# EdwardLiuyc/StaticMapping

Hardware: AMD Instinct MI355X
Metric: scan-pair alignments/sec (120k-pt KITTI-64, 20 ICP iters) (higher is better)
Workload: dtype f32/f64; 1 GPU; BASELINE config #2: IcpFast point-to-plane, 120k-pt synthetic Velodyne-64 scan pair vs CalculateNormals target (~21695 pts), exactly 20 iterations, rho 0.7; 512 distinct consecutive pairs of a synthetic drive (speed 6-10 m/s, yaw rate +-0.2 rad/s, seed 5), guess = previous pair's motion; pairs_per_gpu=512, distinct_pairs=512, target_points_mean=21695, nn_mode=grid, guess=extrapolated, split_after=2, parallelism=pairs round-robin over 1 GPU(s), one RCCL gather of poses, rccl_ranks=1

## Files before the change

### staticmapping_amd/csrc/icp_kernels.hip

```cpp
#include <type_traits>
#include "smhip_device.h"
#include "kd_median_tree.h"
#include "grid_lookup.h"
#include "icp_tail_math.h"

namespace smhip {

__device__ __forceinline__ bool xcd_block(int nblk, int npairs, int b_pair_base, int& pair, int& blk) {
  const int id = blockIdx.x;
  const int j = id >> 3;
  const int local = (j / nblk) * 8 + (id & 7);
  pair = b_pair_base + local;
  blk = j % nblk;
  return local < npairs;
}

__global__ __launch_bounds__(256) void tgt_reduce(IcpDev b) {
  const int pair = b.pair_base + blockIdx.y;
  const int nt = b.in[pair].nt;
  const float4* tp = b.tgt_p + (size_t)pair * b.nt_cap;
  double sx = 0, sy = 0, sz = 0;
  float mn[3] = {INFINITY, INFINITY, INFINITY}, mx[3] = {-INFINITY, -INFINITY, -INFINITY};
  const int chunk = (nt + gridDim.x - 1) / gridDim.x;
  const int lo = blockIdx.x * chunk, hi = min(nt, lo + chunk);
// ... 640 lines not shown
    unsigned long long m[4];
    if (!class_masks(it, m)) continue;
#pragma unroll
    for (int c = 0; c < 4; ++c) tot[c] += (uint32_t)__popcll(m[c]);
  }
  uint32_t basepos[4];
#pragma unroll
  for (int c = 0; c < 4; ++c) {
    uint32_t v = 0;
    if (lane == 0 && tot[c]) v = atomicAdd(&st->nabo_count[c], tot[c]);
    basepos[c] = (uint32_t)__builtin_amdgcn_readlane((int)v, 0);
  }
#pragma unroll
  for (int it = 0; it < ITEMS; ++it) {
    unsigned long long m[4];
    if (!class_masks(it, m)) continue;
    const uint32_t c = (uint32_t)(cls2 >> (2 * it)) & 3u;
    if ((nabo_failed >> it) & 1u) {
      const unsigned long long mine = c == 0 ? m[0] : (c == 1 ? m[1] : (c == 2 ? m[2] : m[3]));
      const uint32_t bp = c == 0 ? basepos[0] : (c == 1 ? basepos[1] : (c == 2 ? basepos[2] : basepos[3]));
      *nabo_list_slot(b, so, (int)c, bp + (uint32_t)__popcll(mine & lt)) = base + it * kNnThreads + (int)threadIdx.x;
    }
#pragma unroll
    for (int c2 = 0; c2 < 4; ++c2) basepos[c2] += (uint32_t)__popcll(m[c2]);
  }
}

template <int ITEMS, bool NABO = false>
__global__ __launch_bounds__(kNnThreads) void nn_certify(IcpDev b, int nblk) {
  int pair, blk;
  if (!xcd_block(nblk, b.npairs, b.pair_base, pair, blk)) return;
  PairState* st = &b.state[pair];
  if (st->done) return;
  const int ns = st->ns;
  const int base = blk * (kNnThreads * ITEMS);
  if (base >= ns) return;
  double Mc[12];
#pragma unroll
  for (int k = 0; k < 12; ++k) Mc[k] = st->M[k];
  const Pot pot = {(float)st->pot_a, (float)st->pot_b, 0.f, 0.f};
  __shared__ uint32_t s_hist[kHistBins];
  for (int k = threadIdx.x; k < kHistBins; k += kNnThreads) s_hist[k] = 0;
  __syncthreads();
  const int lane = threadIdx.x & 63;
  const size_t so = (size_t)pair * b.ns_cap;
  const float4* __restrict__ tq = b.tq + (size_t)pair * b.nt_cap;
  const float r_need = 0.9f * sqrtf(st->rcap2);
  uint32_t min_lb = 0xffffffffu;
  uint32_t nabo_failed = 0;
  int ic = min(base + (int)threadIdx.x, ns - 1);
  float4 s_1 = ld_src(b, so + ic);
  float l_1 = ld_lb(b, so + ic);
  int j_1 = b.idx[so + ic];
  ic = min(base + kNnThreads + (int)threadIdx.x, ns - 1);
  float4 s_2 = ld_src(b, so + ic);
  float l_2 = ld_lb(b, so + ic);
  int j_2 = b.idx[so + ic];
  float4 t_1 = tq[max(j_1, 0)];
  for (int it = 0; it < ITEMS; ++it) {
    const int i = base + it * kNnThreads + threadIdx.x;
    bool hard = false, fail = false;
    const float4 s = s_1;
    const float l = l_1;
    const int j = j_1;
    const float4 t = t_1;
    s_1 = s_2; l_1 = l_2; j_1 = j_2;
    if (it + 1 < ITEMS) t_1 = tq[max(j_1, 0)];
    if (it + 2 < ITEMS) {
      ic = min(i + 2 * kNnThreads, ns - 1);
      s_2 = ld_src(b, so + ic);
      l_2 = ld_lb(b, so + ic);
      j_2 = b.idx[so + ic];
    }
    if (i < ns) {
      double px, py, pz;
      transform_point(Mc, s, px, py, pz);
      const float qx = (float)px, qy = (float)py, qz = (float)pz;
      const float Lp = bound_now(l, pot_at(pot, norm3(s.x, s.y, s.z)));
      fail = true;
      if (NABO) {
        const float Pn = pot_at(pot, norm3(s.x, s.y, s.z));
        if (isfinite(qx) && isfinite(qy) && isfinite(qz) && l > 0.f && j >= 0 &&
            l - Pn - 4.0e-7f * (l + Pn) - 1.3e-7f * (fabsf(qx) + fabsf(qy) + fabsf(qz)) > 0.f) {
          const float d1 = dist2(t, qx, qy, qz);
          b.d2[so + i] = d1;
          atomicAdd(&s_hist[__float_as_uint(d1) >> kHistShift], 1u);
          fail = false;
        }
      } else if (isfinite(qx) && isfinite(qy) && isfinite(qz) && Lp > 0.f) {
        if (l > 0.f && j >= 0) {
          const float d1 = dist2(t, qx, qy, qz);
          if (d1 < Lp * Lp) {
            b.d2[so + i] = d1;
            atomicAdd(&s_hist[__float_as_uint(d1) >> kHistShift], 1u);
            fail = false;
          }
        } else if (l < 0.f && Lp >= r_need) {
          const float lb2 = Lp * Lp;
          b.d2[so + i] = lb2;
          atomicAdd(&s_hist[__float_as_uint(lb2) >> kHistShift], 1u);
          min_lb = min(min_lb, __float_as_uint(lb2));
          hard = true;
          fail = false;
        }
      }
    }
    const unsigned long long dm = __ballot(fail);
    if (NABO) {
      if (fail) nabo_failed |= 1u << it;
    } else if (dm) {
      uint32_t basepos = 0;
      if (lane == 0) basepos = atomicAdd(&st->deferred_count, (uint32_t)__popcll(dm));
      basepos = (uint32_t)__builtin_amdgcn_readlane((int)basepos, 0);
      if (fail) b.dlist[so + basepos + __popcll(dm & ((1ull << lane) - 1ull))] = i;
    }
    const unsigned long long hm = __ballot(hard);
    if (hm) {
      uint32_t basepos = 0;
      if (lane == 0) basepos = atomicAdd(&st->hard_count, (uint32_t)__popcll(hm));
      basepos = (uint32_t)__builtin_amdgcn_readlane((int)basepos, 0);
      if (hard) b.hlist[so + basepos + __popcll(hm & ((1ull << lane) - 1ull))] = i;
    }
  }
  if (NABO) nabo_list_append<ITEMS>(b, st, so, base, ns, nabo_failed, lane);
#pragma unroll
  for (int off = 32; off > 0; off >>= 1) min_lb = min(min_lb, (uint32_t)__shfl_xor((int)min_lb, off, 64));
  if (lane == 0 && min_lb != 0xffffffffu) atomicMin(&st->min_lb_key, min_lb);
  __syncthreads();
  uint32_t* gh = b.hist + (size_t)pair * kHistBins;
  for (int k = threadIdx.x; k < kHistBins; k += kNnThreads) {
    const uint32_t v = s_hist[k];
    if (v) atomicAdd(&gh[k], v);
  }
}

__device__ __forceinline__ void sweep_run(const float4* __restrict__ tq, uint32_t j0, uint32_t j1,
                                          float qx, float qy, float qz, Best& best) {
  uint32_t j = j0;
  for (; j + 4 <= j1; j += 4) {
    const float4 t0 = tq[j], t1 = tq[j + 1], t2 = tq[j + 2], t3 = tq[j + 3];
    test_ascending_ru(t0, (int)j, qx, qy, qz, best);
    test_ascending_ru(t1, (int)j + 1, qx, qy, qz, best);
    test_ascending_ru(t2, (int)j + 2, qx, qy, qz, best);
    test_ascending_ru(t3, (int)j + 3, qx, qy, qz, best);
  }
  for (; j < j1; ++j) test_ascending_ru(tq[j], (int)j, qx, qy, qz, best);
}

#ifndef SMHIP_PHASE_TIMING
#define SMHIP_PHASE_TIMING 0
#endif
#if SMHIP_PHASE_TIMING
#define SMHIP_PHASE(k) do { if (timing) { const unsigned long long now_ = __builtin_readcyclecounter(); tacc[k] += now_ - tprev; tprev = now_; } } while (0)
#else
#define SMHIP_PHASE(k) do { } while (0)
#endif
template <int ITEMS, bool FIRST>
__device__ __forceinline__ void ball_lds_rounds(const IcpDev& b, PairState* st, const PairState* ls, int pair, int base0, const double* Mc,
                                                uint32_t* s_hist, uint32_t& min_lb) {
  const int ns = ls->ns;
  const Pot pot = {(float)ls->pot_a, (float)ls->pot_b, (float)ls->step_a, (float)ls->step_b};
  const float Mtx = (float)Mc[3], Mty = (float)Mc[7], Mtz = (float)Mc[11];
#if SMHIP_PHASE_TIMING
  const bool timing = (b.debug_flags & 16) != 0;
  unsigned long long tacc[8] = {0, 0, 0, 0, 0, 0, 0, 0};
  unsigned long long tprev = timing ? __builtin_readcyclecounter() : 0ull;
#endif
  __shared__ uint32_t s_tab[kLdsTableCap];
  __shared__ float4 s_pts[kLdsPointCap];
  __shared__ uint32_t s_roff[kLdsRowCap + 1];
  __shared__ uint32_t s_occ[kLdsRowCap / 32 + 1];
  __shared__ float4 s_q[kNnThreads];
  __shared__ float s_r2[kNnThreads];
  __shared__ uint16_t s_lid[kNnThreads];
  __shared__ uint32_t s_nsearch[2];
  __shared__ uint32_t s_w[17];
  __shared__ int s_box[2][6];
  if (threadIdx.x < 6) { s_box[0][threadIdx.x] = threadIdx.x < 3 ? 0x3fffffff : -0x3fffffff; s_box[1][threadIdx.x] = s_box[0][threadIdx.x]; }
  if (threadIdx.x < 2) s_nsearch[threadIdx.x] = 0;
  __syncthreads();
  const int lane = threadIdx.x & 63;
  const size_t so = (size_t)pair * b.ns_cap;
  const uint2* __restrict__ words = b.words + (size_t)pair * kMaxGridWords;
  const uint32_t* __restrict__ cstart = b.cstart + (size_t)pair * (b.nt_cap + 1);
  const float4* __restrict__ tq = b.tq + (size_t)pair * b.nt_cap;
  const float ox = ls->origin[0], oy = ls->origin[1], oz = ls->origin[2];
  const float h = ls->h, inv_h = ls->inv_h;
  const int nx = ls->nx, ny = ls->ny, nz = ls->nz, wx = ls->wx, nw = ls->nw;
  const float r2cap = ls->rcap2;
  const float r_need = 0.9f * sqrtf(r2cap);
  const bool have_prev = !FIRST && ls->iter > 0;
  const bool certify = have_prev && b.certify;

  int i = base0 + threadIdx.x;
  float4 s_cur = make_float4(0, 0, 0, 0);
  int jp_cur = -1;
  float l_cur = 0.f;
  if (i < ns) {
    s_cur = ld_src(b, so + i);
    if (have_prev) { jp_cur = b.idx[so + i]; if (certify) l_cur = ld_lb(b, so + i); }
  }

  for (int it = 0; it < ITEMS; ++it) {
    const int base = base0 + it * kNnThreads;
    if (base >= ns) break;
    i = base + threadIdx.x;
    int* box = s_box[it & 1];
    uint32_t* nsearch = &s_nsearch[it & 1];
    const int i_next = i + kNnThreads;
    float4 s_next = make_float4(0, 0, 0, 0);
    int jp_next = -1;
    float l_next = 0.f;
    if (it + 1 < ITEMS && i_next < ns) {
      s_next = ld_src(b, so + i_next);
      if (have_prev) { jp_next = b.idx[so + i_next]; if (certify) l_next = ld_lb(b, so + i_next); }
    }
    SMHIP_PHASE(0);
    float qx = 0.f, qy = 0.f, qz = 0.f;
    bool valid = false;
    if (i < ns) {
      double px, py, pz;
      transform_point(Mc, s_cur, px, py, pz);
      qx = (float)px; qy = (float)py; qz = (float)pz;
      valid = isfinite(qx) && isfinite(qy) && isfinite(qz);
    }
    const bool has_jp = valid && jp_cur >= 0;
    float dub2 = INFINITY;
    if (has_jp) dub2 = dist2(tq[jp_cur], qx, qy, qz);
    bool need_search = valid, hard = false;
    if (i < ns && !valid) {
      b.d2[so + i] = INFINITY; st_match(b, so + i, -1, 0.f);
    }
    const float sn = __builtin_amdgcn_sqrtf(fmaf(s_cur.z, s_cur.z, fmaf(s_cur.y, s_cur.y, s_cur.x * s_cur.x)));
    const float delta = have_prev ? fmaf(pot.sa, sn, pot.sb) : 0.03f;
    if (certify && valid) {
      const float Lp = bound_now(l_cur, pot_at(pot, sn));
      if (Lp > 0.f) {
        if (l_cur > 0.f && has_jp && dub2 < Lp * Lp) {
          b.d2[so + i] = dub2;
          atomicAdd(&s_hist[__float_as_uint(dub2) >> kHistShift], 1u);
          need_search = false;
        } else if (l_cur < 0.f && Lp >= r_need) {
          const float lb2 = Lp * Lp;
          b.d2[so + i] = lb2;
          atomicAdd(&s_hist[__float_as_uint(lb2) >> kHistShift], 1u);
          min_lb = min(min_lb, __float_as_uint(lb2));
          hard = true;
          need_search = false;
        }
      }
    }
    {
      const unsigned long long sm = __ballot(need_search);
      if (sm) {
        uint32_t basepos = 0;
        if (lane == 0) basepos = atomicAdd(nsearch, (uint32_t)__popcll(sm));
        basepos = (uint32_t)__builtin_amdgcn_readlane((int)basepos, 0);
        if (need_search) {
          const uint32_t pos = basepos + __popcll(sm & ((1ull << lane) - 1ull));
          s_q[pos] = make_float4(qx, qy, qz, __int_as_float(jp_cur));
          s_r2[pos] = has_jp ? search_radius2(r2cap, dub2, search_margin(delta)) : r2cap;
          s_lid[pos] = (uint16_t)threadIdx.x;
        }
      }
    }
    {
      const unsigned long long hm = __ballot(hard);
      if (hm) {
        uint32_t basepos = 0;
        if (lane == 0) basepos = atomicAdd(&st->hard_count, (uint32_t)__popcll(hm));
        basepos = (uint32_t)__builtin_amdgcn_readlane((int)basepos, 0);
        if (hard) b.hlist[so + basepos + __popcll(hm & ((1ull << lane) - 1ull))] = i;
      }
    }
    SMHIP_PHASE(1);
    __syncthreads();
    SMHIP_PHASE(2);
    const int nq = (int)*nsearch;
    if (threadIdx.x == 0 && nq) atomicAdd(&st->deferred_count, (uint32_t)nq);
    const bool mine = (int)threadIdx.x < nq;
    float R2 = 0.f;
    int jseed = -1, gi = -1;
    if (mine) {
      const float4 q4 = s_q[threadIdx.x];
      qx = q4.x; qy = q4.y; qz = q4.z; jseed = __float_as_int(q4.w);
      R2 = s_r2[threadIdx.x];
      gi = base + (int)s_lid[threadIdx.x];
    }
    int x0 = 1, x1 = 0, y0 = 1, y1 = 0, z0 = 1, z1 = 0;
    if (mine) {
      const float Rs = __builtin_amdgcn_sqrtf(R2) * 1.0001f + 1.0e-3f * h;
      x0 = max(cell_coord(qx - Rs, ox, inv_h), 0); x1 = min(cell_coord(qx + Rs, ox, inv_h), nx - 1);
      y0 = max(cell_coord(qy - Rs, oy, inv_h), 0); y1 = min(cell_coord(qy + Rs, oy, inv_h), ny - 1);
      z0 = max(cell_coord(qz - Rs, oz, inv_h), 0); z1 = min(cell_coord(qz + Rs, oz, inv_h), nz - 1);
    }
    const bool inbox = mine && x0 <= x1 && y0 <= y1 && z0 <= z1;
    if ((int)(threadIdx.x & ~63) < nq) {
      const int big = 0x3fffffff;
      const int mx0 = wave_min_i(inbox ? x0 : big), mx1 = wave_max_i(inbox ? x1 : -big);
      const int my0 = wave_min_i(inbox ? y0 : big), my1 = wave_max_i(inbox ? y1 : -big);
      const int mz0 = wave_min_i(inbox ? z0 : big), mz1 = wave_max_i(inbox ? z1 : -big);
      if (lane == 0 && mx0 <= mx1) {
        atomicMin(&box[0], mx0); atomicMin(&box[1], my0); atomicMin(&box[2], mz0);
        atomicMax(&box[3], mx1); atomicMax(&box[4], my1); atomicMax(&box[5], mz1);
      }
    }
    SMHIP_PHASE(3);
    __syncthreads();
    const int X0 = box[0], Y0 = box[1], Z0 = box[2];
    const int nxl = box[3] - X0 + 2, nyl = box[4] - Y0 + 1, nzl = box[5] - Z0 + 1;
    const bool any = box[3] >= X0;
    const long long entries = any ? (long long)nxl * nyl * nzl : 0;
    const bool use_lds = any && entries <= kLdsTableCap;
    if (use_lds) {
      const float inv_nxl = 1.0f / (float)nxl, inv_nyl = 1.0f / (float)nyl;
      for (int e = threadIdx.x; e < (int)entries; e += kNnThreads) {
        const int r = (int)(((float)e + 0.5f) * inv_nxl);
        const int x = X0 + (e - r * nxl);
        const int zz = (int)(((float)r + 0.5f) * inv_nyl);
        const int y = Y0 + (r - zz * nyl), z = Z0 + zz;
        const int widx = (z * ny + y) * wx + (x >> 5);
        uint32_t val = (uint32_t)ls->nt;
        if (widx < nw) {
          const uint2 wd = words[widx];
          val = cstart[wd.y + __popc(wd.x & ((1u << (x & 31)) - 1u))];
        }
        s_tab[e] = val;
      }
    }
    if (threadIdx.x < 6) s_box[(it + 1) & 1][threadIdx.x] = threadIdx.x < 3 ? 0x3fffffff : -0x3fffffff;
    if (threadIdx.x == 6) s_nsearch[(it + 1) & 1] = 0;
    const int rows = use_lds ? nyl * nzl : 0;
    bool pts_lds = use_lds && rows <= kLdsRowCap;
    if (use_lds) __syncthreads();
    if (pts_lds) {
      uint32_t len = 0;
      if ((int)threadIdx.x < rows) len = s_tab[threadIdx.x * nxl + nxl - 1] - s_tab[threadIdx.x * nxl];
      {
        const unsigned long long om = __ballot(len > 0);
        if (lane == 0) { s_occ[2 * (threadIdx.x >> 6)] = (uint32_t)om; s_occ[2 * (threadIdx.x >> 6) + 1] = (uint32_t)(om >> 32); }
        if (threadIdx.x == 0) s_occ[kLdsRowCap / 32] = 0u;
      }
      uint32_t total;
      const uint32_t off = block_excl_scan(len, s_w, &total);
      if ((int)threadIdx.x < rows) s_roff[threadIdx.x] = off;
      if (threadIdx.x == 0) s_roff[rows] = total;
      __syncthreads();
      pts_lds = total <= (uint32_t)kLdsPointCap;
      if (pts_lds) {
        for (uint32_t k = threadIdx.x; k < total; k += kNnThreads) {
          int lo = 0, hi = rows - 1;
          while (lo < hi) { const int mid = (lo + hi + 1) >> 1; if (s_roff[mid] <= k) lo = mid; else hi = mid - 1; }
          const uint32_t j = s_tab[lo * nxl] + (k - s_roff[lo]);
          float4 t = tq[j];
          t.w = __int_as_float((int)j);
          s_pts[k] = t;
        }
      }
    }
    __syncthreads();
    SMHIP_PHASE(4);
    bool hard2 = false;
    if (mine) {
      Best best = {INFINITY, -1, INFINITY};
      if (x0 <= x1 && y0 <= y1 && z0 <= z1) {
        const float slack = 2.0e-3f * h;
        const uint32_t ymask = (2u << (y1 - y0)) - 1u;
        for (int z = z0; z <= z1; ++z) {
          const float zl = oz + (float)z * h;
          const float dz = fmaxf(fmaxf(zl - qz, qz - (zl + h)) - slack, 0.f);
          const int ra = (z - Z0) * nyl + (y0 - Y0);
          uint32_t m = ymask;
          if (pts_lds) m &= __builtin_amdgcn_alignbit(s_occ[(ra >> 5) + 1], s_occ[ra >> 5], (uint32_t)(ra & 31));
          while (m) {
            const int bpos = __ffs((int)m) - 1;
            m &= m - 1u;
            const int y = y0 + bpos;
            const float yl = oy + (float)y * h;
            const float dy = fmaxf(fmaxf(yl - qy, qy - (yl + h)) - slack, 0.f);
            if (fmaf(dy, dy, dz * dz) > R2) continue;
            if (pts_lds) {
              const int r = ra + bpos;
              const int rb = r * nxl - X0;
              const uint32_t g0 = s_tab[rb + X0];
              const uint32_t k0 = s_roff[r] + (s_tab[rb + x0] - g0), k1 = s_roff[r] + (s_tab[rb + x1 + 1] - g0);
              for (const float4 *tp = s_pts + k0, *te = s_pts + k1; tp < te; ++tp) {
                const float4 t = *tp;
                test_ascending_ru(t, __float_as_int(t.w), qx, qy, qz, best);
              }
            } else if (use_lds) {
              const int rb = (ra + bpos) * nxl - X0;
              sweep_run(tq, s_tab[rb + x0], s_tab[rb + x1 + 1], qx, qy, qz, best);
            } else {
              uint32_t sb, se;
              row_slots(words, (z * ny + y) * wx, x0, x1, sb, se);
              if (se > sb) sweep_run(tq, cstart[sb], cstart[se], qx, qy, qz, best);
            }
          }
        }
      }
      float d2out, lbout;
      int jout;
      if (best.d2 <= R2) {
        d2out = best.d2;
        jout = best.j;
        lbout = __builtin_amdgcn_sqrtf(fminf(best.s2, R2));
      } else {
        d2out = R2;
        jout = best.j >= 0 ? best.j : jseed;
        lbout = -__builtin_amdgcn_sqrtf(R2);
        hard2 = true;
        min_lb = min(min_lb, __float_as_uint(R2));
      }
      SMHIP_PHASE(5);
      b.d2[so + gi] = d2out;
      {
        const float ux = qx - Mtx, uy = qy - Mty, uz = qz - Mtz;
        st_match(b, so + gi, jout, with_pot(lbout, pot_at(pot, __builtin_amdgcn_sqrtf(fmaf(uz, uz, fmaf(uy, uy, ux * ux))))));
      }
      const uint32_t key = __float_as_uint(d2out);
      if (key < 0x7f800000u) atomicAdd(&s_hist[key >> kHistShift], 1u);
    }
    {
      const unsigned long long hm = __ballot(hard2);
      if (hm) {
        uint32_t basepos = 0;
        if (lane == 0) basepos = atomicAdd(&st->hard_count, (uint32_t)__popcll(hm));
        basepos = (uint32_t)__builtin_amdgcn_readlane((int)basepos, 0);
        if (hard2) b.hlist[so + basepos + __popcll(hm & ((1ull << lane) - 1ull))] = gi;
      }
    }
    s_cur = s_next; jp_cur = jp_next; l_cur = l_next;
    SMHIP_PHASE(6);
  }
#if SMHIP_PHASE_TIMING
  if (timing && lane == 0) {
    unsigned long long* tc = reinterpret_cast<unsigned long long*>(b.tpart);
    for (int k = 0; k < 8; ++k) atomicAdd(&tc[k], tacc[k]);
  }
#endif
}

__device__ __forceinline__ void flush_min_lb(PairState* st, uint32_t min_lb) {
#pragma unroll
  for (int off = 32; off > 0; off >>= 1) min_lb = min(min_lb, (uint32_t)__shfl_xor((int)min_lb, off, 64));
  if ((threadIdx.x & 63) == 0 && min_lb != 0xffffffffu) atomicMin(&st->min_lb_key, min_lb);
}
__device__ __forceinline__ void flush_hist(const IcpDev& b, int pair, const uint32_t* s_hist) {
  __syncthreads();
  uint32_t* gh = b.hist + (size_t)pair * kHistBins;
  for (int k = threadIdx.x; k < kHistBins; k += kNnThreads) {
    const uint32_t v = s_hist[k];
    if (v) atomicAdd(&gh[k], v);
  }
}
__device__ __forceinline__ void flush_min_lb_and_hist(const IcpDev& b, PairState* st, int pair, uint32_t min_lb, const uint32_t* s_hist) {
  flush_min_lb(st, min_lb);
  flush_hist(b, pair, s_hist);
}

template <int ITEMS, bool FIRST = false>
__global__ __launch_bounds__(kNnThreads, 5) void nn_ball_lds(IcpDev b, int nblk) {
  int pair, blk;
  if (!xcd_block(nblk, b.npairs, b.pair_base, pair, blk)) return;
  PairState* st = &b.state[pair];
  if (st->done) return;
  const int base0 = blk * (kNnThreads * ITEMS);
  if (base0 >= st->ns) return;
  double Mc[12];
#pragma unroll
  for (int k = 0; k < 12; ++k) Mc[k] = st->M[k];
  __shared__ uint32_t s_hist[kHistBins];
  for (int k = threadIdx.x; k < kHistBins; k += kNnThreads) s_hist[k] = 0;
  uint32_t min_lb = 0xffffffffu;
  ball_lds_rounds<ITEMS, FIRST>(b, st, st, pair, base0, Mc, s_hist, min_lb);
  flush_min_lb_and_hist(b, st, pair, min_lb, s_hist);
}

__device__ __forceinline__ void listed_append_hard(const IcpDev& b, PairState* st, size_t so, bool hard, int i, int lane);
constexpr int kWaveBoxRows = 1024;
constexpr int kWaveCand = 256;

__device__ __forceinline__ void lane_ball_search(const uint2* __restrict__ words, const uint32_t* __restrict__ cstart, const float4* __restrict__ tq,
                                                 float ox, float oy, float oz, float h, int ny, int wx, float qx, float qy, float qz, float R2,
                                                 int x0, int x1, int y0, int y1, int z0, int z1, Best& best) {
  const float slack = 2.0e-3f * h;
  for (int z = z0; z <= z1; ++z) {
    const float zl = oz + (float)z * h;
    const float dz = fmaxf(fmaxf(zl - qz, qz - (zl + h)) - slack, 0.f);
    for (int y = y0; y <= y1; ++y) {
      const float yl = oy + (float)y * h;
      const float dy = fmaxf(fmaxf(yl - qy, qy - (yl + h)) - slack, 0.f);
      if (fmaf(dy, dy, dz * dz) > R2) continue;
      uint32_t sb, se;
      row_slots(words, (z * ny + y) * wx, x0, x1, sb, se);
      if (se > sb) {
        const uint32_t j0 = cstart[sb], j1 = cstart[se];
        for (uint32_t j = j0; j < j1; ++j) test_ascending_ru(tq[j], (int)j, qx, qy, qz, best);
      }
    }
  }
}
__device__ __forceinline__ void test_pair_ru(const float4 a, const float4 c, float qx, float qy, float qz, Best& best) {
  const f32x2 dx = (f32x2){qx, qx} - (f32x2){a.x, a.y};
  const f32x2 dy = (f32x2){qy, qy} - (f32x2){a.z, a.w};
  const f32x2 dz = (f32x2){qz, qz} - (f32x2){c.x, c.y};
  f32x2 d = dx * dx;
  d = __builtin_elementwise_fma(dy, dy, d);
  d = __builtin_elementwise_fma(dz, dz, d);
  best.s2 = __builtin_amdgcn_fmed3f(d.x, best.d2, best.s2);
  if (d.x < best.d2) { best.d2 = d.x; best.j = __float_as_int(c.z); }
  best.s2 = __builtin_amdgcn_fmed3f(d.y, best.d2, best.s2);
  if (d.y < best.d2) { best.d2 = d.y; best.j = __float_as_int(c.w); }
}

template <int ITEMS, bool FIRST>
__global__ __launch_bounds__(kNnThreads) void nn_ball_wave(IcpDev b, int nblk) {
  int pair, blk;
  if (!xcd_block(nblk, b.npairs, b.pair_base, pair, blk)) return;
  PairState* st = &b.state[pair];
  if (st->done) return;
  const int ns = st->ns;
  const int base0 = blk * (kNnThreads * ITEMS);
  if (base0 >= ns) return;
  double Mc[12];
#pragma unroll
  for (int k = 0; k < 12; ++k) Mc[k] = st->M[k];
  const Pot pot = {(float)st->pot_a, (float)st->pot_b, (float)st->step_a, (float)st->step_b};
  const float Mtx = (float)Mc[3], Mty = (float)Mc[7], Mtz = (float)Mc[11];
  __shared__ uint32_t s_hist[kHistBins];
  __shared__ float4 s_cand[kNnThreads / 64][kWaveCand];
  __shared__ uint32_t s_roff[kNnThreads / 64][64];
  __shared__ uint32_t s_rbase[kNnThreads / 64][64];
  __shared__ uint32_t s_nsearch;
  for (int k = threadIdx.x; k < kHistBins; k += kNnThreads) s_hist[k] = 0;
  if (threadIdx.x == 0) s_nsearch = 0;
  __syncthreads();
  const int lane = threadIdx.x & 63, wave = threadIdx.x >> 6;
  float4* cand = s_cand[wave];
  uint32_t* roff = s_roff[wave];
  uint32_t* rbase = s_rbase[wave];
  const size_t so = (size_t)pair * b.ns_cap;
  const uint2* __restrict__ words = b.words + (size_t)pair * kMaxGridWords;
  const uint32_t* __restrict__ cstart = b.cstart + (size_t)pair * (b.nt_cap + 1);
  const float4* __restrict__ tq = b.tq + (size_t)pair * b.nt_cap;
  const float ox = st->origin[0], oy = st->origin[1], oz = st->origin[2];
  const float h = st->h, inv_h = st->inv_h;
  const int nx = st->nx, ny = st->ny, nz = st->nz, wx = st->wx;
  const float r2cap = st->rcap2;
  const float r_need = 0.9f * sqrtf(r2cap);
  const bool have_prev = !FIRST && st->iter > 0;
  const bool certify = have_prev && b.certify;
  uint32_t min_lb = 0xffffffffu;
  uint32_t nsearch = 0;

  int i = base0 + threadIdx.x;
  float4 s_cur = make_float4(0, 0, 0, 0);
  int jp_cur = -1;
  float l_cur = 0.f;
  if (i < ns) {
    s_cur = ld_src(b, so + i);
    if (have_prev) { jp_cur = b.idx[so + i]; if (certify) l_cur = ld_lb(b, so + i); }
  }
  for (int it = 0; it < ITEMS; ++it) {
    const int base = base0 + it * kNnThreads;
    if (base >= ns) break;
    i = base + threadIdx.x;
    const int i_next = i + kNnThreads;
    float4 s_next = make_float4(0, 0, 0, 0);
    int jp_next = -1;
    float l_next = 0.f;
    if (it + 1 < ITEMS && i_next < ns) {
      s_next = ld_src(b, so + i_next);
      if (have_prev) { jp_next = b.idx[so + i_next]; if (certify) l_next = ld_lb(b, so + i_next); }
    }
    float qx = 0.f, qy = 0.f, qz = 0.f;
    bool valid = false;
    if (i < ns) {
      double px, py, pz;
      transform_point(Mc, s_cur, px, py, pz);
      qx = (float)px; qy = (float)py; qz = (float)pz;
      valid = isfinite(qx) && isfinite(qy) && isfinite(qz);
    }
    const bool has_jp = valid && jp_cur >= 0;
    float dub2 = INFINITY;
    if (has_jp) dub2 = dist2(tq[jp_cur], qx, qy, qz);
    bool need_search = valid, hard = false;
    if (i < ns && !valid) {
      b.d2[so + i] = INFINITY; st_match(b, so + i, -1, 0.f);
    }
    float R2 = r2cap;
// ... 1585 lines not shown
#pragma unroll
    for (int off = 1; off < 64; off <<= 1) { const int v = __shfl_up(incl, off, 64); if (lane >= off) incl += v; }
    s_pre[wv][2 * lane] = (uint32_t)(incl - ca - cb);
    s_pre[wv][2 * lane + 1] = (uint32_t)(incl - cb);
    const int e1 = __shfl(incl, 63, 64);
    __syncthreads();
    for (int eb = 0; eb < e1; eb += 64 * kU) {
      int i[kU], jm[kU];
      float d[kU];
      float4 s4[kU], q4[kU], n4[kU];
      bool live[kU], below[kU], rec[kU];
#pragma unroll
      for (int u = 0; u < kU; ++u) {
        const int r = eb + 64 * u + lane;
        live[u] = r < e1;
        i[u] = 0;
        if (live[u]) {
          int wd = 0;
#pragma unroll
          for (int step = kWords / 2; step > 0; step >>= 1) if ((int)s_pre[wv][wd + step] <= r) wd += step;
          uint32_t w = s_bits[wv][wd];
          for (int t = r - (int)s_pre[wv][wd]; t > 0; --t) w &= w - 1u;
          i[u] = wave * range + p0 + wd * 32 + (__ffs(w) - 1);
        }
      }
#pragma unroll
      for (int u = 0; u < kU; ++u) { d[u] = b.d2[so + i[u]]; jm[u] = b.idx[so + i[u]]; s4[u] = ld_src(b, so + i[u]); }
#pragma unroll
      for (int u = 0; u < kU; ++u) {
        const uint32_t key = __float_as_uint(d[u]);
        const int bin = (int)(key >> kHistShift);
        const bool valid = live[u] && key < 0x7f800000u && jm[u] >= 0;
        below[u] = valid && bin < band_lo;
        rec[u] = valid && bin >= band_lo && bin <= band_hi;
        if (below[u]) { q4[u] = b.tq[to + jm[u]]; n4[u] = b.tn[to + jm[u]]; }
      }
#pragma unroll
      for (int u = 0; u < kU; ++u) {
        if (below[u]) accumulate_terms(Mc, s4[u], q4[u], n4[u], acc);
        const unsigned long long bm = __ballot(rec[u]);
        if (rec[u]) {
          const size_t at = segbase + wcount + __popcll(bm & ((1ull << lane) - 1ull));
          b.rec_a[at] = make_float4(s4[u].x, s4[u].y, s4[u].z, d[u]);
          b.rec_j[at] = jm[u];
        }
        wcount += (int)__popcll(bm);
      }
    }
    __syncthreads();
  }
  if (lane == 0) b.gcount[(size_t)pair * b.seg_stride + nseg0 + wave] = (uint32_t)wcount;
  block_reduce29(acc, s_red, s_out);
  if (threadIdx.x < 29) b.partials[((size_t)pair * b.part_stride + nblk0 + blk) * kAccCols + threadIdx.x] = s_out[threadIdx.x];
}


struct TailOpts {
  float cap_factor, ball_radius, band_gain, band_pad;
  int32_t fused, early_exit, max_iteration;
  uint32_t* search_hist;
  uint32_t* done_count;
};
template <class B>
__device__ __forceinline__ uint32_t finalize_tail(const B& b, PairState* st, int pair, const double* s_tot, uint32_t n_valid, uint32_t limit_key,
                                                  bool fusedm, int ns, bool publish) {
  st->fallback_total += st->unresolved_count;
  st->unresolved_count = 0;
  st->hard_total += st->hard_count;
  st->hard_count = 0;
  {
    const uint32_t walked = st->nabo_count[0] + st->nabo_count[1] + st->nabo_count[2] + st->nabo_count[3];
    const uint32_t searched = st->iter == 0 ? (uint32_t)ns : (walked ? walked : (st->deferred_count ? st->deferred_count : (uint32_t)ns));
    st->searched_total += searched;
    if (publish && st->iter < kSearchHist) b.search_hist[(size_t)pair * kSearchHist + st->iter] = searched;
    for (int c = 0; c < 4; ++c) st->nabo_count[c] = 0;
  }
  const uint32_t n_listed = st->deferred_count;
  st->deferred_count = 0;
  st->min_lb_key = 0xffffffffu;
  st->refine = 0;
  {
    const float lim = sqrtf(__uint_as_float(limit_key));
    float rc = fminf(fmaxf(b.cap_factor * lim, 0.05f), b.ball_radius);
    if (!(n_valid > 0)) rc = b.ball_radius;
    st->rcap2 = rc * rc;
  }
  {
    const uint32_t prev = st->limit_key;
    int lo = 0, hi = -1;
    if (n_valid > 0 && prev != 0u && limit_key != 0u) {
      const double x = (double)limit_key;
      const double w = fmax((double)b.band_gain * fabs(x - (double)prev), (double)b.band_pad * 1048576.0);
      const double l = x - w, u = x + w;
      if (l >= 1048576.0 && u < 2139095040.0) { lo = (int)((uint32_t)l >> kHistShift); hi = (int)((uint32_t)u >> kHistShift); }
      if (hi - lo > 2) { lo = 0; hi = -1; }
      if (b.fused && n_listed > (uint32_t)kFusedListedMax) { lo = 0; hi = -1; }
    }
    st->band_lo = lo; st->band_hi = hi;
    if (fusedm) st->spec_hits += 1;
    st->spec_ok = 0;
  }
  st->limit_key = limit_key;
  const double kept = s_tot[28];
  st->kept = (int)kept;
  if (n_valid == 0 || kept < 1.0) {
    st->status = 6;
    st->done = 1;
    for (int c = 0; c < 4; ++c) for (int r = 0; r < 4; ++r) st->result[4 * c + r] = st->guess[4 * r + c];
    st->score = 0;
    if (publish) atomicAdd(b.done_count, 1u);
    return n_listed;
  }
  double A[36], rhs[6], x[6];
  {
    int c = 0;
#pragma unroll
    for (int a = 0; a < 6; ++a)
#pragma unroll
      for (int e = a; e < 6; ++e) { A[6 * a + e] = s_tot[c]; A[6 * e + a] = s_tot[c]; ++c; }
#pragma unroll
    for (int a = 0; a < 6; ++a) rhs[a] = -s_tot[21 + a];
  }
  solve6(A, rhs, x);
  double dT[16] = {1, 0, 0, 0, 0, 1, 0, 0, 0, 0, 1, 0, 0, 0, 0, 1};
  angle_axis_step(x, dT);
  double Tn[16];
  mat4_mul_rm(dT, st->T_iter, Tn);
  for (int i = 0; i < 16; ++i) st->T_iter[i] = Tn[i];
  double Mn[16];
  mat4_mul_rm(Tn, st->G, Mn);
  motion_potential_step(Mn, st->M, &st->step_a, &st->step_b);
  st->pot_a += st->step_a; st->pot_b += st->step_b;
  for (int i = 0; i < 12; ++i) { st->M_prev[i] = st->M[i]; st->M[i] = Mn[i]; }
  const int it = ++st->iter;
  const bool converged = history_push_converged(st->quat, st->trans, &st->n_hist, Tn, b.early_exit != 0);
  if (converged || it >= b.max_iteration) {
    double Tm[16] = {1, 0, 0, st->mu[0], 0, 1, 0, st->mu[1], 0, 0, 1, st->mu[2], 0, 0, 0, 1};
    double Rm[16];
    mat4_mul_rm(Tm, Mn, Rm);
    for (int c = 0; c < 4; ++c) for (int r = 0; r < 4; ++r) st->result[4 * c + r] = Rm[4 * r + c];
    st->done = 1;
    if (publish) atomicAdd(b.done_count, 1u);
  }
  return n_listed;
}

template <bool COMP>
__device__ __forceinline__ void finalize_body(const IcpDev& b) {
  const int pair = b.pair_base + blockIdx.x;
  PairState* st = &b.state[pair];
  if (st->done) return;
#if SMHIP_PHASE_TIMING
  if ((b.debug_flags & 16) && pair == 0 && threadIdx.x == 0) {
    unsigned long long* tc = reinterpret_cast<unsigned long long*>(b.tpart);
    unsigned long long tot = 0;
    for (int k = 0; k < 8; ++k) tot += tc[k];
    printf("[phase] iter %d total %llu :", st->iter, tot);
    for (int k = 0; k < 8; ++k) { printf(" %.1f%%", tot ? 100.0 * (double)tc[k] / (double)tot : 0.0); tc[k] = 0; }
    printf("\n");
  }
#endif
  __shared__ uint32_t s_w[17];
  __shared__ uint32_t s_q[4];
  __shared__ uint32_t s_h[256];
  __shared__ uint32_t s_sel[2];
  __shared__ double s_red[4][29];
  __shared__ double s_tot[29];
  __shared__ double s_part[8][32];
  __shared__ uint32_t s_keys[kFinalizeKeyCap];
  uint32_t* gh = b.hist + (size_t)pair * kHistBins;
#if SMHIP_PHASE_TIMING
  const bool ftime = (b.debug_flags & 32) && threadIdx.x == 0;
  unsigned long long fstamp[8];
  int fk = 0;
#define SMHIP_FPH() do { if (ftime && fk < 8) fstamp[fk++] = wall_clock64(); } while (0)
#else
#define SMHIP_FPH() do { } while (0)
#endif
  SMHIP_FPH();
  find_quantile_bin(gh, b.rho, s_w, s_q);
  SMHIP_FPH();
  const uint32_t qbin = s_q[0], below = s_q[1], n_valid = s_q[2], krank = s_q[3];
  const int ns = st->ns;
  const bool fusedm = b.fused && st->spec_ok;
  const int chunk = fusedm ? kNnThreads * kCertifyItems : kAccThreads * ((b.fused && !b.fused_nabo) ? b.sums_items : b.acc_items);
  const int nblk = (ns + chunk - 1) / chunk;
  const int nseg0 = nblk * 4;
  const int seg_len0 = chunk / 4;
  const bool nabof = fusedm && b.fused_nabo;
  constexpr int kNaboSegs = kNaboAccBlocks * (kAccThreads / 64);
  const int nseg = nseg0 + (fusedm ? (nabof ? kNaboSegs : (int)b.litems[pair]) : 0);
  const int seg_len1 = nabof ? b.bl_stride / kNaboSegs : kNnThreads >> listed_lanes_log2((int)st->deferred_count, b.listed_lane_budget);
  const int nrows = nblk + (fusedm ? (nabof ? kNaboAccBlocks : (int)((st->deferred_count + (uint32_t)kListedSumChunk - 1u) / (uint32_t)kListedSumChunk)) : 0);
  constexpr int kPrefRows = 8;
  double pref[kPrefRows];
  {
    const double* part = b.partials + (size_t)pair * b.part_stride * kAccCols + (threadIdx.x & 31);
#pragma unroll
    for (int u = 0; u < kPrefRows; ++u) {
      const int k = (int)(threadIdx.x >> 5) + 8 * u;
      pref[u] = k < nrows ? part[(size_t)k * kAccCols] : 0.0;
    }
  }
  const uint32_t* gcount = b.gcount + (size_t)pair * b.seg_stride;
  const float4* ra = b.rec_a + (size_t)pair * 2 * b.bl_stride;
  const int32_t* rj = b.rec_j + (size_t)pair * 2 * b.bl_stride;
  __shared__ uint32_t s_off[2 * kFinalizeMaxSeg];
  auto rec_at = [&](int sg, int k) -> uint32_t {
    return sg < nseg0 ? (uint32_t)(sg * seg_len0 + k) : (uint32_t)(b.bl_stride + (sg - nseg0) * seg_len1 + k);
  };
  auto segment_of = [&](int e) -> int {
    int lo = 0, hi = nseg - 1;
    while (lo < hi) {
      const int mid = (lo + hi + 1) >> 1;
      if (s_off[mid] <= (uint32_t)e) lo = mid; else hi = mid - 1;
    }
    return lo;
  };
  auto member = [&](int e) -> uint32_t {
    const int sg = segment_of(e);
    return rec_at(sg, e - (int)s_off[sg]);
  };
  double acc[29];
#pragma unroll
  for (int c = 0; c < 29; ++c) acc[c] = 0.0;
  SMHIP_FPH();
  uint32_t limit_key = 0;
  int nb = 0;
  bool flat = false;
  int top = 1;
  if (n_valid > 0) {
    const int per = (nseg + 255) >> 8;
    const int s0 = (int)threadIdx.x * per;
    uint32_t c[kFinalizeMaxSeg / 256];
    uint32_t mine = 0;
#pragma unroll
    for (int k = 0; k < kFinalizeMaxSeg / 256; ++k) {
      c[k] = (k < per && s0 + k < nseg) ? gcount[s0 + k] : 0u;
      mine += c[k];
    }
    uint32_t total;
    uint32_t o = block_excl_scan(mine, s_w, &total);
#pragma unroll
    for (int k = 0; k < kFinalizeMaxSeg / 256; ++k)
      if (k < per && s0 + k < nseg) { s_off[s0 + k] = o; o += c[k]; }
    while (2 * top < nseg) top *= 2;
    for (int x = nseg + (int)threadIdx.x; x < 2 * top; x += 256) s_off[x] = 0xffffffffu;
    nb = (int)total;
    flat = nb <= kFinalizeKeyCap;
    __syncthreads();
    if (flat && nb > 0) {
      constexpr int kPer = 16;
      for (int r0 = 0; r0 < nb; r0 += kPer * 256) {
        int sg[kPer];
        uint32_t pos[kPer];
        float4 aa[kPer];
#pragma unroll
        for (int k = 0; k < kPer; ++k) sg[k] = 0;
        for (int step = top; step > 0; step >>= 1) {
#pragma unroll
          for (int k = 0; k < kPer; ++k) {
            const int cand = sg[k] + step;
            sg[k] = s_off[cand] <= (uint32_t)min(r0 + (int)threadIdx.x + 256 * k, nb - 1) ? cand : sg[k];
          }
        }
#pragma unroll
        for (int k = 0; k < kPer; ++k) pos[k] = rec_at(sg[k], min(r0 + (int)threadIdx.x + 256 * k, nb - 1) - (int)s_off[sg[k]]);
#pragma unroll
        for (int k = 0; k < kPer; ++k) aa[k] = ra[pos[k]];
#pragma unroll
        for (int k = 0; k < kPer; ++k) {
          const int e = r0 + (int)threadIdx.x + 256 * k;
          if (e < nb) s_keys[e] = __float_as_uint(aa[k].w);
        }
      }
    }
    __syncthreads();
  }
  SMHIP_FPH();
  if (n_valid > 0) {
    uint32_t rank = krank - below;
    uint32_t prefix = 0, mask = 0;
    const int shifts[3] = {12, 4, 0};
    const int widths[3] = {8, 8, 4};
    for (int pass = 0; pass < 3; ++pass) {
      const int shift = shifts[pass];
      const uint32_t nd = 1u << widths[pass];
      s_h[threadIdx.x] = 0;
      __syncthreads();
      for (int e = threadIdx.x; e < nb; e += blockDim.x) {
        const uint32_t full = flat ? s_keys[e] : __float_as_uint(ra[member(e)].w);
        const uint32_t key = full & 0xfffffu;
        if ((full >> kHistShift) == qbin && (key & mask) == prefix) atomicAdd(&s_h[(key >> shift) & (nd - 1u)], 1u);
      }
      __syncthreads();
      {
        const uint32_t v = threadIdx.x < nd ? s_h[threadIdx.x] : 0u;
        uint32_t tot;
        const uint32_t excl = block_excl_scan(v, s_w, &tot);
        if (threadIdx.x == 0) { s_sel[0] = nd - 1; s_sel[1] = tot - s_h[nd - 1]; }
        __syncthreads();
        if (v > 0 && excl <= rank && rank < excl + v) { s_sel[0] = threadIdx.x; s_sel[1] = excl; }
      }
      __syncthreads();
      prefix |= s_sel[0] << shift;
      mask |= (nd - 1u) << shift;
      rank -= s_sel[1];
      __syncthreads();
    }
    limit_key = (qbin << kHistShift) | prefix;
    SMHIP_FPH();
    const size_t to = (size_t)pair * b.nt_cap;
// ... 150 lines not shown
```

Before: 26970 alignments/s.

## Compact deferred NN searches across all items before running dense search rounds

In non-first iterations the ball search now runs every query round first and appends all points that need a real search into one block-wide compaction buffer sized ITEMS*kNnThreads. The grid searches then run over dense batches of kNnThreads entries, so there are fewer sparsely populated search rounds and fewer barriers per item. The first iteration searches each round directly without staging. The change also drops the stored seed index, re-reading b.idx on the fallback path, and extends the optional phase-timing counters. The cost is more LDS per block, which may lower occupancy.

```diff
diff --git a/staticmapping_amd/csrc/icp_kernels.hip b/staticmapping_amd/csrc/icp_kernels.hip
--- a/staticmapping_amd/csrc/icp_kernels.hip
+++ b/staticmapping_amd/csrc/icp_kernels.hip
@@ -816,6 +816,9 @@
 #endif
 #if SMHIP_PHASE_TIMING
 #define SMHIP_PHASE(k) do { if (timing) { const unsigned long long now_ = __builtin_readcyclecounter(); tacc[k] += now_ - tprev; tprev = now_; } } while (0)
+__device__ __forceinline__ unsigned long long* phase_counter(const IcpDev& b, int k) {
+  return reinterpret_cast<unsigned long long*>(b.tpart) + (k / 7) * 16 + 9 + (k % 7);
+}
 #else
 #define SMHIP_PHASE(k) do { } while (0)
 #endif
@@ -827,21 +830,26 @@
   const float Mtx = (float)Mc[3], Mty = (float)Mc[7], Mtz = (float)Mc[11];
 #if SMHIP_PHASE_TIMING
   const bool timing = (b.debug_flags & 16) != 0;
-  unsigned long long tacc[8] = {0, 0, 0, 0, 0, 0, 0, 0};
+  unsigned long long tacc[14] = {0, 0, 0, 0, 0, 0, 0, 0, 0, 0, 0, 0, 0, 0};
   unsigned long long tprev = timing ? __builtin_readcyclecounter() : 0ull;
 #endif
   __shared__ uint32_t s_tab[kLdsTableCap];
   __shared__ float4 s_pts[kLdsPointCap];
   __shared__ uint32_t s_roff[kLdsRowCap + 1];
   __shared__ uint32_t s_occ[kLdsRowCap / 32 + 1];
-  __shared__ float4 s_q[kNnThreads];
-  __shared__ float s_r2[kNnThreads];
-  __shared__ uint16_t s_lid[kNnThreads];
-  __shared__ uint32_t s_nsearch[2];
   __shared__ uint32_t s_w[17];
   __shared__ int s_box[2][6];
+  float4* s_e = nullptr;
+  uint16_t* s_slot = nullptr;
+  uint32_t* s_nsearch = nullptr;
+  if constexpr (!FIRST) {
+    __shared__ float4 s_e_[ITEMS * kNnThreads];
+    __shared__ uint16_t s_slot_[ITEMS * kNnThreads];
+    __shared__ uint32_t s_nsearch_;
+    s_e = s_e_; s_slot = s_slot_; s_nsearch = &s_nsearch_;
+    if (threadIdx.x == 6) s_nsearch_ = 0;
+  }
   if (threadIdx.x < 6) { s_box[0][threadIdx.x] = threadIdx.x < 3 ? 0x3fffffff : -0x3fffffff; s_box[1][threadIdx.x] = s_box[0][threadIdx.x]; }
-  if (threadIdx.x < 2) s_nsearch[threadIdx.x] = 0;
   __syncthreads();
   const int lane = threadIdx.x & 63;
   const size_t so = (size_t)pair * b.ns_cap;
@@ -865,12 +873,10 @@
     if (have_prev) { jp_cur = b.idx[so + i]; if (certify) l_cur = ld_lb(b, so + i); }
   }
 
-  for (int it = 0; it < ITEMS; ++it) {
+  auto query_round = [&](const int it, float& qx, float& qy, float& qz, bool& valid) -> bool {
     const int base = base0 + it * kNnThreads;
-    if (base >= ns) break;
+    if (base >= ns) return false;
     i = base + threadIdx.x;
-    int* box = s_box[it & 1];
-    uint32_t* nsearch = &s_nsearch[it & 1];
     const int i_next = i + kNnThreads;
     float4 s_next = make_float4(0, 0, 0, 0);
     int jp_next = -1;
@@ -880,8 +886,8 @@
       if (have_prev) { jp_next = b.idx[so + i_next]; if (certify) l_next = ld_lb(b, so + i_next); }
     }
     SMHIP_PHASE(0);
-    float qx = 0.f, qy = 0.f, qz = 0.f;
-    bool valid = false;
+    qx = 0.f; qy = 0.f; qz = 0.f;
+    valid = false;
     if (i < ns) {
       double px, py, pz;
       transform_point(Mc, s_cur, px, py, pz);
@@ -914,17 +920,16 @@
         }
       }
     }
-    {
+    if constexpr (!FIRST) {
       const unsigned long long sm = __ballot(need_search);
       if (sm) {
         uint32_t basepos = 0;
-        if (lane == 0) basepos = atomicAdd(nsearch, (uint32_t)__popcll(sm));
+        if (lane == 0) basepos = atomicAdd(s_nsearch, (uint32_t)__popcll(sm));
         basepos = (uint32_t)__builtin_amdgcn_readlane((int)basepos, 0);
         if (need_search) {
           const uint32_t pos = basepos + __popcll(sm & ((1ull << lane) - 1ull));
-          s_q[pos] = make_float4(qx, qy, qz, __int_as_float(jp_cur));
-          s_r2[pos] = has_jp ? search_radius2(r2cap, dub2, search_margin(delta)) : r2cap;
-          s_lid[pos] = (uint16_t)threadIdx.x;
+          s_e[pos] = make_float4(qx, qy, qz, has_jp ? search_radius2(r2cap, dub2, search_margin(delta)) : r2cap);
+          s_slot[pos] = (uint16_t)(it * kNnThreads + (int)threadIdx.x);
         }
       }
     }
@@ -937,20 +942,15 @@
         if (hard) b.hlist[so + basepos + __popcll(hm & ((1ull << lane) - 1ull))] = i;
       }
     }
+    s_cur = s_next; jp_cur = jp_next; l_cur = l_next;
     SMHIP_PHASE(1);
-    __syncthreads();
-    SMHIP_PHASE(2);
-    const int nq = (int)*nsearch;
-    if (threadIdx.x == 0 && nq) atomicAdd(&st->deferred_count, (uint32_t)nq);
-    const bool mine = (int)threadIdx.x < nq;
-    float R2 = 0.f;
-    int jseed = -1, gi = -1;
-    if (mine) {
-      const float4 q4 = s_q[threadIdx.x];
-      qx = q4.x; qy = q4.y; qz = q4.z; jseed = __float_as_int(q4.w);
-      R2 = s_r2[threadIdx.x];
-      gi = base + (int)s_lid[threadIdx.x];
-    }
+    return true;
+  };
+  auto search_round = [&](const int sr, const bool mine, const bool wave_live, const float qx, const float qy, const float qz, const float R2, const int gi) {
+    int* box = s_box[sr & 1];
+#if SMHIP_PHASE_TIMING
+    const unsigned long long tround = timing ? __builtin_readcyclecounter() : 0ull;
+#endif
     int x0 = 1, x1 = 0, y0 = 1, y1 = 0, z0 = 1, z1 = 0;
     if (mine) {
       const float Rs = __builtin_amdgcn_sqrtf(R2) * 1.0001f + 1.0e-3f * h;
@@ -959,7 +959,7 @@
       z0 = max(cell_coord(qz - Rs, oz, inv_h), 0); z1 = min(cell_coord(qz + Rs, oz, inv_h), nz - 1);
     }
     const bool inbox = mine && x0 <= x1 && y0 <= y1 && z0 <= z1;
-    if ((int)(threadIdx.x & ~63) < nq) {
+    if (wave_live) {
       const int big = 0x3fffffff;
       const int mx0 = wave_min_i(inbox ? x0 : big), mx1 = wave_max_i(inbox ? x1 : -big);
       const int my0 = wave_min_i(inbox ? y0 : big), my1 = wave_max_i(inbox ? y1 : -big);
@@ -992,8 +992,7 @@
         s_tab[e] = val;
       }
     }
-    if (threadIdx.x < 6) s_box[(it + 1) & 1][threadIdx.x] = threadIdx.x < 3 ? 0x3fffffff : -0x3fffffff;
-    if (threadIdx.x == 6) s_nsearch[(it + 1) & 1] = 0;
+    if (threadIdx.x < 6) s_box[(sr + 1) & 1][threadIdx.x] = threadIdx.x < 3 ? 0x3fffffff : -0x3fffffff;
     const int rows = use_lds ? nyl * nzl : 0;
     bool pts_lds = use_lds && rows <= kLdsRowCap;
     if (use_lds) __syncthreads();
@@ -1071,7 +1070,7 @@
         lbout = __builtin_amdgcn_sqrtf(fminf(best.s2, R2));
       } else {
         d2out = R2;
-        jout = best.j >= 0 ? best.j : jseed;
+        jout = best.j >= 0 ? best.j : (have_prev ? b.idx[so + gi] : -1);
         lbout = -__builtin_amdgcn_sqrtf(R2);
         hard2 = true;
         min_lb = min(min_lb, __float_as_uint(R2));
@@ -1094,13 +1093,50 @@
         if (hard2) b.hlist[so + basepos + __popcll(hm & ((1ull << lane) - 1ull))] = gi;
       }
     }
-    s_cur = s_next; jp_cur = jp_next; l_cur = l_next;
     SMHIP_PHASE(6);
+#if SMHIP_PHASE_TIMING
+    if (timing) {
+      const unsigned long long dt = __builtin_readcyclecounter() - tround, one = threadIdx.x < 64 ? 1ull : 0ull;
+      if (pts_lds) { tacc[8] += one; tacc[9] += dt; }
+      else if (use_lds) { tacc[10] += one; tacc[11] += dt; }
+      else { tacc[12] += one; tacc[13] += dt; }
+    }
+#endif
+  };
+  if constexpr (FIRST) {
+    uint32_t nvalid = 0;
+    for (int it = 0; it < ITEMS; ++it) {
+      float qx, qy, qz;
+      bool valid;
+      if (!query_round(it, qx, qy, qz, valid)) break;
+      const unsigned long long vm = __ballot(valid);
+      nvalid += (uint32_t)__popcll(vm);
+      SMHIP_PHASE(2);
+      search_round(it, valid, vm != 0ull, qx, qy, qz, r2cap, base0 + it * kNnThreads + (int)threadIdx.x);
+    }
+    if (lane == 0 && nvalid) atomicAdd(&st->deferred_count, nvalid);
+  } else {
+    for (int it = 0; it < ITEMS; ++it) {
+      float qx, qy, qz;
+      bool valid;
+      if (!query_round(it, qx, qy, qz, valid)) break;
+    }
+    __syncthreads();
+    SMHIP_PHASE(2);
+    const int nq = (int)*s_nsearch;
+    if (threadIdx.x == 0 && nq) atomicAdd(&st->deferred_count, (uint32_t)nq);
+    for (int sr = 0, e0 = 0; e0 < nq; ++sr, e0 += kNnThreads) {
+      const int e = e0 + (int)threadIdx.x;
+      const bool mine = e < nq;
+      float4 q4 = make_float4(0.f, 0.f, 0.f, 0.f);
+      int gi = -1;
+      if (mine) { q4 = s_e[e]; gi = base0 + (int)s_slot[e]; }
+      search_round(sr, mine, (e & ~63) < nq, q4.x, q4.y, q4.z, q4.w, gi);
+    }
   }
 #if SMHIP_PHASE_TIMING
   if (timing && lane == 0) {
-    unsigned long long* tc = reinterpret_cast<unsigned long long*>(b.tpart);
-    for (int k = 0; k < 8; ++k) atomicAdd(&tc[k], tacc[k]);
+    for (int k = 0; k < 14; ++k) atomicAdd(phase_counter(b, k), tacc[k]);
   }
 #endif
 }
@@ -2992,12 +3028,16 @@
   if (st->done) return;
 #if SMHIP_PHASE_TIMING
   if ((b.debug_flags & 16) && pair == 0 && threadIdx.x == 0) {
-    unsigned long long* tc = reinterpret_cast<unsigned long long*>(b.tpart);
+    unsigned long long tc[14];
+    for (int k = 0; k < 14; ++k) { tc[k] = *phase_counter(b, k); *phase_counter(b, k) = 0; }
     unsigned long long tot = 0;
     for (int k = 0; k < 8; ++k) tot += tc[k];
     printf("[phase] iter %d total %llu :", st->iter, tot);
-    for (int k = 0; k < 8; ++k) { printf(" %.1f%%", tot ? 100.0 * (double)tc[k] / (double)tot : 0.0); tc[k] = 0; }
-    printf("\n");
+    for (int k = 0; k < 8; ++k) printf(" %.1f%%", tot ? 100.0 * (double)tc[k] / (double)tot : 0.0);
+    const unsigned long long ptot = tc[9] + tc[11] + tc[13];
+    printf(" | search rounds: staged %llu (%.1f%% of their cycles), table only %llu (%.1f%%), global %llu (%.1f%%); rounds' share of all cycles %.1f%%\n",
+           tc[8], ptot ? 100.0 * (double)tc[9] / (double)ptot : 0.0, tc[10], ptot ? 100.0 * (double)tc[11] / (double)ptot : 0.0,
+           tc[12], ptot ? 100.0 * (double)tc[13] / (double)ptot : 0.0, tot ? 100.0 * (double)ptot / (double)tot : 0.0);
   }
 #endif
   __shared__ uint32_t s_w[17];
```

After: 28080 alignments/s, median of 6. 4.1% higher.
